# hpgmg/hpgmg

Hardware: AMD Instinct MI355X
Metric: DOF/s (fine-grid) for FMG F-cycle (higher is better)
Workload: dtype f64

## Files before the change

### hpgmg_amd/csrc/host/mg.c

```c
#include <stdio.h>
#include <stdlib.h>
#include <string.h>
#include <math.h>
#include <time.h>
#include <stdint.h>
#include "hpgmg_level.h"
#include "hpgmg_operators.h"
#include "hpgmg_mg.h"

hpgmg_solve_record hpgmg_last_solve;
int hpgmg_verbose = 1;

void hpgmg_communicator_free(communicator_type *C);

static double now(void) {
  struct timespec ts;
  clock_gettime(CLOCK_MONOTONIC, &ts);
  return (double)ts.tv_sec + 1e-9 * (double)ts.tv_nsec;
}
#define SAY(rank, ...) do { if ((rank) == 0 && hpgmg_verbose) { fprintf(stdout, __VA_ARGS__); fflush(stdout); } } while (0)

typedef struct { int send_rank, send_id, send_box, recv_rank, recv_id, recv_box, i, j, k; } xfer_t;

static int xfer_cmp(const void *pa, const void *pb) {
// ... 632 lines not shown
}
void MGPreconditionerApply(mg_type *G, int onLevel, int z_id, int r_id, double a, double b) {
  level_type *L = G->levels[onLevel];
  if (!L->active) return;
  L->vcycles_from_this_level++;
  zero_vector(L, z_id);
  MGVCycle(G, z_id, r_id, a, b, onLevel);
  seg_close();
}

static int hpgmg_fmg_vcycles = 0;
void hpgmg_set_fmg_vcycles(int n) { hpgmg_fmg_vcycles = n > 0 ? n : 0; }
static int fmg_zero_u_first = 0;
void hpgmg_fmg_zero_u_first(void) { fmg_zero_u_first = 1; }
static void fmg_solve_once(mg_type *G, int onLevel, int u_id, int F_id, double a, double b, double rtol);
void FMGSolve(mg_type *G, int onLevel, int u_id, int F_id, double a, double b, double rtol) {
  int attempt, l, booked[64];
  for (attempt = 0; attempt < 2; attempt++) {
    for (l = 0; l < G->num_levels && l < 64; l++) booked[l] = G->levels[l]->vcycles_from_this_level;
    hpgmg_solve_attempt_begin();
    fmg_solve_once(G, onLevel, u_id, F_id, a, b, rtol);
    if (!hpgmg_solve_attempt_end()) return;
    G->MGSolves_performed--;
    for (l = 0; l < G->num_levels && l < 64; l++) G->levels[l]->vcycles_from_this_level = booked[l];
    if (G->levels[onLevel]->active) zero_vector(G->levels[onLevel], u_id);
  }
  fprintf(stderr, "hpgmg: FMGSolve failed twice\n");
  exit(1);
}
static void fmg_solve_once(mg_type *G, int onLevel, int u_id, int F_id, double a, double b, double rtol) {
  const int e_id = u_id, R_id = VECTOR_R, maxVCycles = hpgmg_fmg_vcycles;
  const int bottom = G->num_levels - 1;
  level_type *L = G->levels[onLevel];
  char label[64];
  int l, v;
  int u_to_zero = fmg_zero_u_first;
  hpgmg_tick t;
  fmg_zero_u_first = 0;
  G->MGSolves_performed++;
  if (!L->active) return;
  SAY(L->my_rank, "FMGSolve... ");
  const double t0 = now();
  seg_reset(G, onLevel, u_id, F_id, a, b);

  t = hpgmg_tick_begin(L, &L->timers.Total, "norm(F), R = F");
  double norm_of_F = 0.0;
  int first_restriction = onLevel;
  int norm_deferred = 0;
  const hpgmg_fmg_hook *hook = fmg_hook;
  if (!hook && onLevel < bottom && hpgmg_norm_scale_restrict_fused_deferred(L, F_id, R_id, G->levels[onLevel + 1])) { first_restriction = onLevel + 1; norm_deferred = 1; }
  else if (!hook && onLevel < bottom && hpgmg_norm_scale_restrict_fused(L, F_id, R_id, G->levels[onLevel + 1], &norm_of_F)) first_restriction = onLevel + 1;
  else {
    norm_of_F = norm(L, F_id);
    scale_vector(L, R_id, 1.0, F_id);
  }
  hpgmg_tick_end(t);

  int ftail = bottom;
  for (l = onLevel; l < bottom && !hook; l++) if (is_small(G, l) && hpgmg_vcycle_legs_fused(&G->levels[l], G->num_levels - l, e_id, R_id, a, b, HPGMG_LEG_FCYCLE_TAIL_ASK)) { ftail = l; break; }

  if (u_to_zero && ftail <= onLevel) { zero_vector(L, u_id); u_to_zero = 0; }
  for (l = first_restriction; l < ftail; l++) {
    if (is_small(G, l)) seg_open();
    t = hpgmg_tick_begin(G->levels[l], &G->levels[l]->timers.Total, "restrict R");
    restriction(G->levels[l + 1], R_id, G->levels[l], R_id, RESTRICT_CELL);
    if (hook) hook->rhs_restricted(hook, G, l + 1, R_id);
    hpgmg_tick_end(t);
  }

  if (ftail < bottom) {
    if (is_small(G, ftail)) seg_open();
    t = hpgmg_tick_begin(G->levels[ftail], &G->levels[ftail]->timers.Total, "F-cycle tail (fused)");
    if (!hpgmg_vcycle_legs_fused(&G->levels[ftail], G->num_levels - ftail, e_id, R_id, a, b, HPGMG_LEG_FCYCLE_TAIL)) { fprintf(stderr, "fused F-cycle tail refused after being accepted\n"); exit(1); }
    hpgmg_tick_end(t);
// ... 79 lines not shown
```

### hpgmg_amd/csrc/host/operators_hip.c

```c
#include "plugin_internal.h"

void hp_do_restriction(level_type *Lc, int id_c, level_type *Lf, int id_f, int type) {
  TICK(Lf, restriction_total, "restriction");
  hp_coef_written(Lc, id_c);
  communicator_type *S = &Lf->restriction[type], *R = &Lc->restriction[type];
  backend_t *Bc = hp_backend_of(Lc), *Bf = hp_backend_of(Lf);
  HIP_OK(hpgmg_hip_restrict_blocks(&Bc->dev, id_c, &Bf->dev, id_f, hp_mirror(Lf, S->blocks[0], S->num_blocks[0]), S->num_blocks[0], type));
  hp_transport_phase(R, S, (Lf->tag << 4) | 0x5);
  HIP_OK(hpgmg_hip_restrict_blocks(&Bc->dev, id_c, &Bf->dev, id_f, hp_mirror(Lf, S->blocks[1], S->num_blocks[1]), S->num_blocks[1], type));
  HIP_OK(hpgmg_hip_copy_blocks(&Bc->dev, id_c, hp_mirror(Lc, R->blocks[2], R->num_blocks[2]), R->num_blocks[2]));
  TOCK();
}

int hpgmg_restrict_zero_fused(level_type *Lc, int id_c, level_type *Lf, int id_f, int zero_id) {
  communicator_type *S = &Lf->restriction[RESTRICT_CELL], *R = &Lc->restriction[RESTRICT_CELL];
  if (!Lf->active || !Lc->active || Lc->num_my_boxes < 1 || zero_id == id_c) return 0;
  if (S->num_sends || R->num_recvs || S->num_blocks[0] || R->num_blocks[2] || S->num_blocks[1] < 1) return 0;
  TICK(Lf, restriction_total, "restriction + zero_vector");
  backend_t *Bc = hp_backend_of(Lc), *Bf = hp_backend_of(Lf);
  HIP_OK(hpgmg_hip_restrict_cell_and_zero(&Bc->dev, id_c, &Bf->dev, id_f, hp_mirror(Lf, S->blocks[1], S->num_blocks[1]), S->num_blocks[1], zero_id));
  TOCK();
  return 1;
}

// ... 125 lines not shown
    if (B) { TICK(L, blas1, "norm(F), this rank's part (reduction deferred)"); HIP_OK(hpgmg_hip_norm_max(&B->dev, F_id, &v)); TOCK(); }
    hp_do_scale_vector(L, R_id, 1.0, F_id);
    hp_do_restriction(Lc, R_id, L, R_id, RESTRICT_CELL);
    deferred_host_value = v; deferred_on_device = 0;
  }
  deferred_norm_level = L;
  return 1;
}
double hpgmg_norm_deferred_fetch(level_type *L) {
  double v = deferred_host_value;
  if (deferred_norm_level != L) { fprintf(stderr, "hpgmg: no deferred norm is pending on this level\n"); abort(); }
  deferred_norm_level = NULL;
  if (deferred_on_device) HIP_OK(hpgmg_hip_deferred_fetch(&v));
  return hp_allreduce_scalar(L, v, HPGMG_REDUCE_MAX);
}
int hpgmg_residual_norm_fused(level_type *L, int res_id, int x_id, int rhs_id, double a, double b, double *norm_out) {
  hpgmg_config cfg;
  hpgmg_get_config(&cfg);
  if (cfg.op != HPGMG_OP_7PT && res_id >= 0) return 0;
  if (!L->active || L->num_my_boxes < 1) return 0;
  backend_t *B = hp_backend_of(L);
  const int ready = fused_residual_operand(L, B, x_id);
  if (!ready) return 0;
  double v = 0.0;
  { TICK(L, residual, "residual + norm (fused)");
    FUSED_LAUNCH(B, ready, hpgmg_hip_residual_norm(hp_stencil_dev(B), hp_variant(), res_id, x_id, rhs_id, a, b, 1.0 / (L->h * L->h), &v));
    TOCK(); }
  *norm_out = hp_allreduce_scalar(L, v, HPGMG_REDUCE_MAX);
  return 1;
}
// ... 129 lines not shown
```

### hpgmg_amd/csrc/host/plugin_internal.h

```cpp
#ifndef HPGMG_PLUGIN_INTERNAL_H
#define HPGMG_PLUGIN_INTERNAL_H
#include <stdio.h>
#include <stdlib.h>
#include <string.h>
#include <math.h>
#include <time.h>
#include <stdint.h>
#include "hpgmg_level.h"
#include "hpgmg_operators.h"
#include "hpgmg_mg.h"
#include "hpgmg_hip.h"

int hpgmg_smooth_sweeps(void);
int hpgmg_gsrb_out_of_place(void);

#define HP_INTERNAL __attribute__((visibility("hidden")))

enum { TIMERS_HOST = 0, TIMERS_DEVICE = 1, TIMERS_SYNC = 2 };
#define TICK(L, FIELD, WHAT) const hpgmg_tick tick_ = hpgmg_tick_begin((L), &(L)->timers.FIELD, WHAT)
#define TOCK() hpgmg_tick_end(tick_)
HP_INTERNAL void hp_lazy_flush(void);
#define HIP_OK(call) do { hp_lazy_flush(); int e_ = (call); if (e_) { fprintf(stderr, "hpgmg: %s failed (%d): %s\n", #call, e_, hpgmg_hip_last_error()); abort(); } } while (0)

#define MAX_LISTS 32
// ... 56 lines not shown
  double *storage, *scratch;
  double **d_box_base, **d_pair_base; int *d_box_low, *d_box_nbr;
  hpgmg_hip_level dev, dev_all;
  image_plan plan[IMG_PLANS];
  double *sendbuf, *recvbuf; size_t send_cap, recv_cap;
  double **ptr_tmp; int ptr_cap;
  hpgmg_hip_bc_entry *d_bc; int n_bc, n_bc_own;
  hpgmg_hip_bc_entry *d_bc_k; int n_bc_k;
  int *d_special; int n_special;
  int coef_valid, shape;
  double *seen_v0; int seen_nv;
} halo_images;

typedef enum { SW_GHOST_FREE = 0, SW_ONE_LAUNCH_GHOSTS, SW_OVERLAP, SW_PAIR_REMOTE, SW_IMAGES, SW_FUSED_SWEEPS, SW_PAIR_MIN_CELLS, SW_FUSED_RESIDUAL, SW_FUSED_TAIL,
               SW_FUSED_FTAIL, SW_FUSED_BOTTOM, SW_SMALL_FUSED, SW_SMALL_VTAIL, SW_SMALL_27PT_GSRB, SW_SMALL_OPS, SW_LAZY, SW_LAZY_REPORT, SW_TEMP_SCRATCH,
               SW_FV4_NO_EXACT_RB, SW_GRAPH, SW_SMOOTHER_PRECISION, SW_DEFER_NORM, SW_BRICK_VISITS, SW_BRICK_SIZE, SW_BRICK_MIN_DIM, SW_BRICK_FSTEP, SW_BRICK_CHAIN, SW_BRICK_WIDE, SW_BRICK_WIDE_MAX_DIM, SW_BRICK_WIDE_TAIL_DIM, SW_FTAIL_MAX_DIM, SW_PAIR_FORM_DINV, SW_UNIFORM_ALPHA, SW_COUNT } hp_switch_id;
HP_INTERNAL long long hp_switch(hp_switch_id id);
HP_INTERNAL void hp_switch_set(hp_switch_id id, long long value);

HP_INTERNAL backend_t *hp_backend_of(level_type *L);
HP_INTERNAL const blockCopy_type *hp_mirror(level_type *owner, const blockCopy_type *host, int n);
HP_INTERNAL int  hp_variant(void);
typedef struct { int kind, zero_first; } hp_small_bc;
HP_INTERNAL hp_small_bc hp_small_bc_rule(int op, const level_type *L);
HP_INTERNAL int  hp_boxes_lexicographic(level_type *L);
static inline int hp_comm_no_messages(const communicator_type *C) { return C->num_sends + C->num_recvs == 0 && !C->num_blocks[0] && !C->num_blocks[2]; }
static inline int hp_comm_nothing_to_exchange(const communicator_type *C) { return hp_comm_no_messages(C) && !C->num_blocks[1]; }
HP_INTERNAL int *hp_krylov_pinned(backend_t *B);
HP_INTERNAL int  hp_ghost_free_mode(void);
HP_INTERNAL backend_t *hp_pcg_backend(level_type *L);
HP_INTERNAL int  hp_box_rank_at(const level_type *L, int bi, int bj, int bk);
// ... 85 lines not shown
```

### hpgmg_amd/csrc/host/plugin_switches.c

```c
#include "plugin_internal.h"

enum { K_ON = 0, K_OFF = 1, K_INT = 2, K_TRI = 3 };
static struct { const char *env; int kind; long long dflt; const char *what; long long value; int known; } table[SW_COUNT] = {
  [SW_GHOST_FREE]        = { "HPGMG_GHOST_FREE", K_ON, 1, "stencil launches read neighbouring boxes and the Dirichlet rule themselves; 0: the reference's exchange + boundary + stencil launches" },
  [SW_ONE_LAUNCH_GHOSTS] = { "HPGMG_ONE_LAUNCH_GHOSTS", K_ON, 1, "27-pt / fv2 / fv4: box-to-box ghost copies and boundary conditions as one launch" },
  [SW_OVERLAP]           = { "HPGMG_OVERLAP", K_ON, 1, "N > 1: halo exchanges on a second stream under the part of the stencil launch that does not need them" },
  [SW_PAIR_REMOTE]       = { "HPGMG_PAIR_REMOTE", K_ON, 1, "N > 1, 7-pt: sweep pairs across rank boundaries (two-deep halo, one exchange per pair); 0: one exchange per sweep" },
  [SW_IMAGES]            = { "HPGMG_IMAGES", K_ON, 1, "N > 1, 27-pt / fv4: images of the neighbouring ranks' boxes (one-pass red + black kernels keep running); 0: exchange_boundary per half sweep" },
  [SW_FUSED_SWEEPS]      = { "HPGMG_FUSED_SWEEPS", K_ON, 1, "7-pt: two smoother sweeps per pass on bandwidth-bound levels" },
  [SW_PAIR_MIN_CELLS]    = { "HPGMG_PAIR_MIN_CELLS", K_INT, 2000000, "7-pt: smallest level (cells) that takes the sweep-pair kernel (2 M: the 128^3 level too, since the kernel picks its launch shape per launch -- 16 workgroup rows of 10 waves x 16 chunks = 256 workgroups there: config 2 2.70 vs 2.74 ms; with 16 waves it lost, 3.02 vs 2.92: profiles/r06k_ab_pair_min.txt, r06n_ab_pair_min.txt)" },
  [SW_FUSED_RESIDUAL]    = { "HPGMG_FUSED_RESIDUAL", K_ON, 1, "residual + restriction (+ zero_vector), residual + norm, norm + copy + restriction as one pass each" },
  [SW_FUSED_TAIL]        = { "HPGMG_FUSED_TAIL", K_ON, 1, "7-pt: the V-cycle below the brick levels (<= 8^3; <= 16^3 without them) as one single-workgroup launch" },
  [SW_FUSED_FTAIL]       = { "HPGMG_FUSED_FTAIL", K_ON, 1, "7-pt: the F-cycle's own work below 32^3 as one launch" },
  [SW_FUSED_BOTTOM]      = { "HPGMG_FUSED_BOTTOM", K_ON, 1, "BiCGStab bottom solve on the device; 0: driven from the host (host/solvers.c) through the operators" },
  [SW_SMALL_FUSED]       = { "HPGMG_SMALL_FUSED", K_TRI, 2, "27-pt / fv2 / fv4: smooth() of a one-box level as one launch on an LDS image (2, default); 0 off" },
  [SW_SMALL_VTAIL]       = { "HPGMG_SMALL_VTAIL", K_TRI, 2, "27-pt / fv2 / fv4: the V-cycle below a one-box level as one launch: 2 on except for 27-pt GSRB (default), 1 on, 0 off" },
  [SW_SMALL_27PT_GSRB]   = { "HPGMG_TUNE_SMALL_27PT_GSRB", K_OFF, 0, "27-pt GSRB: the one-launch small-level smooth() instead of the one-workgroup-per-box red + black kernel" },
  [SW_SMALL_OPS]         = { "HPGMG_SMALL_OPS", K_ON, 1, "BLAS-1 / operator calls of a host-driven Krylov solver on a small one-box level go out with the scalar that follows them" },
  [SW_LAZY]              = { "HPGMG_LAZY", K_ON, 1, "void operators are postponed while they follow MGVCycle's call order and issued fused (the reference's own driver, INTEGRATION.md Route B)" },
  [SW_LAZY_REPORT]       = { "HPGMG_LAZY_REPORT", K_OFF, 0, "print what the operator queue did when the process ends" },
  [SW_TEMP_SCRATCH]      = { "HPGMG_TEMP_SCRATCH", K_ON, 1, "inside a cycle VECTOR_TEMP is scratch after smooth(): in-cycle smoother forms; 0: the exact state of smooth() everywhere" },
  [SW_FV4_NO_EXACT_RB]   = { "HPGMG_TUNE_FV4_NO_EXACT_RB", K_OFF, 0, "fv4: the exported smooth() as six half sweeps (no red + black passes)" },
  [SW_GRAPH]             = { "HPGMG_GRAPH", K_OFF, 0, "capture / replay the launch-bound segments as hipGraphs (measured slower with a full stream)" },
  [SW_DEFER_NORM]        = { "HPGMG_DEFER_NORM", K_ON, 1, "FMGSolve: norm(F) of the opening pass is collected at the end, where it is used, instead of waited for at the start" },
  [SW_BRICK_VISITS]     = { "HPGMG_BRICK_VISITS", K_ON, 1, "7-pt: the 64^3 / 32^3 / 16^3 levels of a V-cycle leg as one launch of 8^3 bricks that trade faces, residuals and corrections inside the launch; 0 when other processes run such launches on the same GPU" },
  [SW_BRICK_SIZE]       = { "HPGMG_TUNE_BRICK", K_INT, 8, "side of those bricks: 8 (512 lanes, one cell each) or 16 (1024 lanes, four cells each)" },
  [SW_BRICK_MIN_DIM]    = { "HPGMG_TUNE_BRICK_MIN", K_INT, 16, "smallest level (cells per side) visited as bricks; the levels below it are the single-workgroup tail's" },
  [SW_BRICK_FSTEP]      = { "HPGMG_TUNE_BRICK_FSTEP", K_ON, 1, "FMGSolve: interpolation_fcycle onto a brick level rides in the first launch of the V-cycle that follows it" },
  [SW_BRICK_CHAIN]      = { "HPGMG_TUNE_BRICK_CHAIN", K_INT, 1, "consecutive brick levels of a V-cycle leg in ONE launch (what passes between the levels passes inside it); 0: one launch per level visit" },
  [SW_BRICK_WIDE]       = { "HPGMG_BRICK_WIDE", K_ON, 1, "27-pt / fv4: the same for the operators with wide stencils (kernels/brick_wide.hip: halo of the stencil's radius, apply_BCs_p2 / _v4 on the LDS image)" },
  [SW_BRICK_WIDE_MAX_DIM] = { "HPGMG_TUNE_BRICK_WIDE_MAX", K_INT, 64, "largest level (cells per side) the 27-pt / fv4 plugins visit as bricks (measured: fv4 `7 64` 29.71 / 29.91 / 30.15 ms with 64 / 32 / 16, 27-pt 12.27 / 12.51 / 12.52)" },
  [SW_BRICK_WIDE_TAIL_DIM] = { "HPGMG_TUNE_BRICK_WIDE_TAIL", K_INT, 1, "27-pt / fv4: the largest one-box level left to the single-workgroup tail (1: the 8^3, 4^3 (and 27-pt: 2^3) levels are visited as ONE brick each and only the bottom solve is left; 2 / 4 / 8: the tail starts there)" },
  [SW_FTAIL_MAX_DIM]    = { "HPGMG_TUNE_FTAIL_MAX", K_INT, 8, "7-pt: the largest level (cells per side) the single-launch F-cycle tail starts from (8: the 16^3 step of the climb is a brick launch each way, eight CUs instead of one: config 1 0.320 vs 0.328 ms with 16, config 2 the same within noise; profiles/r06i_ab_ftail.txt)" },
  [SW_PAIR_FORM_DINV]    = { "HPGMG_PAIR_FORM_DINV", K_ON, 1, "7-pt sweep pairs (fp64 streams, one rank, variable coefficients, 10 / 12 waves): Dinv is formed in registers from the coefficient streams instead of read, where VECTOR_DINV is known to be rebuild_operator's output for the same a, b; 0: always read" },
  [SW_UNIFORM_ALPHA]     = { "HPGMG_UNIFORM_ALPHA", K_ON, 1, "7-pt Helmholtz, one rank: where rebuild_operator found alpha to be one bit pattern over the level's interior, the sweep pairs that form Dinv and the wide fused residual passes take it from their arguments instead of streaming VECTOR_ALPHA; 0: always read" },
  [SW_SMOOTHER_PRECISION]= { "HPGMG_SMOOTHER_PRECISION", K_INT, 64, "32: fp32 coefficient streams in the Chebyshev sweep pairs (BASELINE config 5: within 2e-4 of the fp64 norms, and bit-exact against the CPU oracle's fp32 mode, which rounds the same coefficients); 64: bit-exact" },
};

long long hp_switch(hp_switch_id id) {
  if (!table[id].known) {
    const char *e = getenv(table[id].env);
    long long v = table[id].dflt;
    switch (table[id].kind) {
      case K_ON:  v = !(e && e[0] == '0'); break;
      case K_OFF: v = (e && e[0] == '1'); break;
      case K_INT: if (e && *e) v = atoll(e); break;
      default:    v = (e && e[0] == '0') ? 0 : ((e && e[0] == '1') ? 1 : table[id].dflt); break;
    }
    table[id].value = v; table[id].known = 1;
  }
// ... 11 lines not shown
```

### hpgmg_amd/csrc/kernels/blas1.hip

```cpp
#include "reduce.hpp"
#include "knobs.hpp"
#include "launch_dispatch.hpp"

namespace hpgmg {

constexpr int kRowsPerBlock = 4;

struct RowIter {
  int box, j, k;
};
__device__ __forceinline__ bool row_of(int row, int side, int num_boxes, RowIter &r) {
  const int per_box = side * side;
  if (row >= per_box * num_boxes) return false;
  r.box = row / per_box;
  const int rem = row - r.box * per_box;
  r.k = rem / side;
  r.j = rem - r.k * side;
  return true;
}
static inline int rows_grid(int rows) { return (rows + kRowsPerBlock - 1) / kRowsPerBlock; }

enum { OP_AXPBY = 0, OP_MUL, OP_INVERT, OP_SCALE, OP_SHIFT, OP_COLOR, OP_RANDOM };
struct EwArgs { int id_c, id_a, id_b; double sa, sb; int colors, ic, jc, kc; };

// ... 108 lines not shown
    for (int ci = lane; ci < half; ci += 64) {
      const double2 a = *reinterpret_cast<const double2 *>(f + 2 * ci), b = *reinterpret_cast<const double2 *>(f + 2 * ci + jS);
      const double2 cc = *reinterpret_cast<const double2 *>(f + 2 * ci + kS), d = *reinterpret_cast<const double2 *>(f + 2 * ci + jS + kS);
      const double2 ra = make_double2(1.0 * a.x, 1.0 * a.y), rb = make_double2(1.0 * b.x, 1.0 * b.y);
      const double2 rc = make_double2(1.0 * cc.x, 1.0 * cc.y), rd = make_double2(1.0 * d.x, 1.0 * d.y);
      store_pair<NT>(r + 2 * ci, ra); store_pair<NT>(r + 2 * ci + jS, rb);
      store_pair<NT>(r + 2 * ci + kS, rc); store_pair<NT>(r + 2 * ci + jS + kS, rd);
      double v = ra.x + ra.y; v = v + rb.x; v = v + rb.y; v = v + rc.x; v = v + rc.y; v = v + rd.x; v = v + rd.y;
      c[ci] = v * 0.125;
      double q;
      q = fabs(a.x); m = (q > m) ? q : m;  q = fabs(a.y); m = (q > m) ? q : m;  q = fabs(b.x); m = (q > m) ? q : m;  q = fabs(b.y); m = (q > m) ? q : m;
      q = fabs(cc.x); m = (q > m) ? q : m; q = fabs(cc.y); m = (q > m) ? q : m; q = fabs(d.x); m = (q > m) ? q : m;  q = fabs(d.y); m = (q > m) ? q : m;
    }
  }
  block_max_store(m, partials, blockIdx.x);
}

template <bool kFinish>
__global__ __launch_bounds__(64) void tile_sum_kernel(const hpgmg_hip_level L, int id_a, int id_b, double *partials, ResultSlot *result, unsigned long long seq) {
  __shared__ double part[64];
  const int tiles_side = (L.dim + BLOCKCOPY_TILE_J - 1) / BLOCKCOPY_TILE_J;
  const int tiles_per_box = tiles_side * tiles_side;
  const int ntiles = tiles_per_box * L.num_boxes;
  const int t = blockIdx.x * 64 + threadIdx.x;
  if (kFinish) part[threadIdx.x] = 0.0;
  if (t >= ntiles) { if (kFinish) __syncthreads(); return; }
  const int box = t / tiles_per_box, rem = t % tiles_per_box;
  const int k0 = (rem / tiles_side) * BLOCKCOPY_TILE_K, j0 = (rem % tiles_side) * BLOCKCOPY_TILE_J;
  const int k1 = min(k0 + BLOCKCOPY_TILE_K, L.dim), j1 = min(j0 + BLOCKCOPY_TILE_J, L.dim);
  const double *pa = vec_origin(L, box, id_a);
// ... 157 lines not shown
      Aii[i] = 1.0 / d;
    }
  }
  block_max_store(best, partials, blockIdx.x);
}

template <int OP>
static int launch_ew(const hpgmg_hip_level *L, const EwArgs &A) {
  HPGMG_SKIP_IF_REPLAY();
  if (L->num_boxes <= 0) return 0;
  const int rows = L->num_boxes * L->dim * L->dim;
  hipLaunchKernelGGL((elementwise_kernel<OP>), dim3(rows_grid(rows)), dim3(256), 0, g_stream, *L, A);
  HPGMG_LAUNCH_CHECK("elementwise_kernel");
  return 0;
}

}
using namespace hpgmg;

extern "C" {
int hpgmg_hip_graph_flush(void);

int hpgmg_hip_fill(const hpgmg_hip_level *L, int id, double v) {
  HPGMG_SKIP_IF_REPLAY();
  if (L->num_boxes <= 0) return 0;
  const int side = L->dim + 2 * L->ghosts, rows = L->num_boxes * side * side;
  hipLaunchKernelGGL(fill_kernel, dim3(rows_grid(rows)), dim3(256), 0, g_stream, *L, id, v);
  HPGMG_LAUNCH_CHECK("fill_kernel");
  return 0;
}
// ... 36 lines not shown
  if (int e = hpgmg_hip_graph_flush()) return e;
  if (norm_out) *norm_out = 0.0;
  if (L->num_boxes <= 0 || Lc->num_boxes <= 0 || (L->dim & 1) || !(L->flags & 1) || (L->jStride & 1) || (L->kStride & 1) || (L->volume & 1) || f_id == r_id)
    return record_error(hipErrorInvalidValue, "norm_copy_restrict: level not supported");
  const int nblk = rows_grid(L->num_boxes * (L->dim / 2) * (L->dim / 2));
  double *partials = reduction_scratch(nblk);
  if (!partials) return record_error(hipErrorOutOfMemory, "norm_copy_restrict: no scratch");
  if (knob(K_COPY_NT) && (double)L->num_boxes * L->dim * L->dim * L->dim * sizeof(double) > 256e6)
    hipLaunchKernelGGL(norm_copy_restrict_kernel<true>, dim3(nblk), dim3(256), 0, g_stream, *L, f_id, r_id, *Lc, rc_id, map, partials);
  else hipLaunchKernelGGL(norm_copy_restrict_kernel<false>, dim3(nblk), dim3(256), 0, g_stream, *L, f_id, r_id, *Lc, rc_id, map, partials);
  HPGMG_LAUNCH_CHECK("norm_copy_restrict");
  if (!norm_out) return 0;
  if (!deferred) return max_of_partials(nblk, 0.0, norm_out);
  if (int e = scalar_begin(&g_deferred, true)) return e;
  return max_of_partials(nblk, 0.0, g_deferred);
}
int hpgmg_hip_norm_max(const hpgmg_hip_level *L, int id, double *out) {
  if (int e = hpgmg_hip_graph_flush()) return e;
  *out = 0.0;
  if (L->num_boxes <= 0) return 0;
  const int nblk = rows_grid(L->num_boxes * L->dim * L->dim);
  if (nblk <= 64) {
    Scalar t;
    if (int e = scalar_begin(&t)) return e;
    hipLaunchKernelGGL(absmax_small_kernel, dim3(1), dim3(256), 0, g_stream, *L, id, t.slot, t.seq);
    HPGMG_LAUNCH_CHECK("norm_max");
    return scalar_wait(t, out);
  }
  int per_box = rows_grid(L->dim * L->dim);
  while (per_box > 1 && (long long)per_box * L->num_boxes > 4096) per_box = (per_box + 1) / 2;
// ... 76 lines not shown
```

### include/hpgmg_fv.h

```cpp
#ifndef HPGMG_FV_H
#define HPGMG_FV_H

#include "hpgmg_level.h"
#include "hpgmg_operators.h"
#include "hpgmg_mg.h"

#ifdef __cplusplus
extern "C" {
#endif

typedef struct hpgmg_solver {
  level_type level_h;
  mg_type    mg;
  double a, b, h;
  int boxes_in_i, box_dim;
  int my_rank, num_ranks;
} hpgmg_solver;

int hpgmg_choose_boxes_in_i(int log2_box_dim, int target_boxes_per_rank, int num_ranks);

hpgmg_solver *hpgmg_solver_create(int log2_box_dim, int target_boxes_per_rank, int bc, int my_rank, int num_ranks);
hpgmg_solver *hpgmg_solver_create_explicit(int boxes_in_i, int box_dim, int bc, int my_rank, int num_ranks);
void hpgmg_solver_destroy(hpgmg_solver *s);

// ... 89 lines not shown
long long   hpgmg_small_ops_prefetched(void);
void        hpgmg_set_fused_bottom(int on);
void        hpgmg_set_fused_tail(int on);
void        hpgmg_set_brick_visits(int on);
long long   hpgmg_brick_visits(void);
long long   hpgmg_brick_failures(void);
long long   hpgmg_brick_capacity_refusals(void);
void        hpgmg_set_brick_wide(int on);
void        hpgmg_set_brick_chains(int on);
long long   hpgmg_pair_remote_smooths(void);
long long   hpgmg_fp32_pair_smooths(void);
void        hpgmg_set_pair_form_dinv(int on);
long long   hpgmg_pair_formed_dinv_launches(void);
void        hpgmg_set_uniform_alpha(int on);
long long   hpgmg_uniform_alpha_launches(void);
long long   hpgmg_fused_residuals_remote(void);
long long   hpgmg_fv4_rb_smooths(void);
long long   hpgmg_rb27_passes(void);
long long   hpgmg_image_exchanges(void);
void        hpgmg_level_timers(level_type *level, double out[9]);
void        hpgmg_set_gather_dim(int dim);
long long   hpgmg_overlap_count(void);
void        hpgmg_set_overlap(int on);
void        hpgmg_set_smoother_precision(int bits);
int         hpgmg_get_smoother_precision(void);
void        hpgmg_set_graphs(int on);
void        hpgmg_set_fused_sweeps(int on);
void        hpgmg_set_pair_min_cells(long long cells);
void        hpgmg_set_ghost_free(int on);
void        hpgmg_set_box_alignment(int jstride, int kstride, int volume, int base_bytes);
// ... 6 lines not shown
```

### include/hpgmg_hip.h

```cpp
#ifndef HPGMG_HIP_H
#define HPGMG_HIP_H

#include <stddef.h>
#include "hpgmg_level.h"

#ifdef __cplusplus
extern "C" {
#endif

typedef struct {
  double *const *box_base;
  const int *box_low;
  int num_boxes;
  int dim, ghosts, jStride, kStride, volume;
  int dim_i, dim_j, dim_k;
  int periodic;
  const int *box_nbr;
  int flags;
  long long box_stride;
} hpgmg_hip_level;

enum { HPGMG_HIP_7PT_VC_HELMHOLTZ = 0, HPGMG_HIP_7PT_VC_POISSON = 1, HPGMG_HIP_7PT_CC = 2,
       HPGMG_HIP_27PT_CC = 3, HPGMG_HIP_FV4_VC_HELMHOLTZ = 4, HPGMG_HIP_FV4_VC_POISSON = 5 };

// ... 153 lines not shown
                                 const blockCopy_type *blocks, int num_blocks, int order);

int hpgmg_hip_fill(const hpgmg_hip_level *L, int id, double interior_value);
int hpgmg_hip_axpby(const hpgmg_hip_level *L, int id_c, double sa, int id_a, double sb, int id_b);
int hpgmg_hip_mul(const hpgmg_hip_level *L, int id_c, double s, int id_a, int id_b);
int hpgmg_hip_invert(const hpgmg_hip_level *L, int id_c, double s, int id_a);
int hpgmg_hip_scale(const hpgmg_hip_level *L, int id_c, double s, int id_a);
int hpgmg_hip_shift(const hpgmg_hip_level *L, int id_c, int id_a, double shift);
int hpgmg_hip_color(const hpgmg_hip_level *L, int id, int colors, int ic, int jc, int kc);
int hpgmg_hip_random(const hpgmg_hip_level *L, int id);
int hpgmg_hip_norm_max(const hpgmg_hip_level *L, int id, double *out);
int hpgmg_hip_dot(const hpgmg_hip_level *L, int id_a, int id_b, double *out);
int hpgmg_hip_norm_copy_restrict(const hpgmg_hip_level *L, int f_id, int r_id, const hpgmg_hip_level *Lc, int rc_id, const int *map, double *norm_out);
int  hpgmg_hip_norm_copy_restrict_deferred(const hpgmg_hip_level *L, int f_id, int r_id, const hpgmg_hip_level *Lc, int rc_id, const int *restrict_map);
int  hpgmg_hip_deferred_fetch(double *out);
int hpgmg_hip_sum(const hpgmg_hip_level *L, int id, double *out);
int hpgmg_hip_gram(const hpgmg_hip_level *L, const int *id_A, int rows, const int *id_B, int cols, double *C_host);
int hpgmg_hip_pcg_supported(const hpgmg_hip_level *L, int variant);
int hpgmg_hip_pcg_apply_dot(const hpgmg_hip_level *L, int variant, int Ap_id, int p_id, double a, double b, double h2inv, double *dot);
int hpgmg_hip_pcg_update(const hpgmg_hip_level *L, int x_id, int r_id, int p_id, int Ap_id, double alpha, double *rmax);
int hpgmg_hip_pcg_dot(const hpgmg_hip_level *L, int a_id, int b_id, double *dot);
int hpgmg_hip_pcg_dot2(const hpgmg_hip_level *L, int a_id, int c_id, int b_id, double *ab, double *cb);
#define HPGMG_HIP_BLOCK_TILE 6
int hpgmg_hip_block_supported(const hpgmg_hip_level *L);
int hpgmg_hip_block_tile(void);
int hpgmg_hip_block_gram(const hpgmg_hip_level *L, const int *a_ids, int na, const int *b_ids, int nb, int w_id, double *G_host);
int hpgmg_hip_block_combine(const hpgmg_hip_level *L, const int *out_ids, int nout, const int *in_ids, int nin, const double *C_host);
int hpgmg_hip_block_residual(const hpgmg_hip_level *L, const int *r_ids, const int *ax_ids, const int *x_ids, int n, int w_id, const double *mu,
                             double *rmax, double *mxmax);

// ... 96 lines not shown
```

### include/hpgmg_operators.h

```cpp
#ifndef HPGMG_OPERATORS_H
#define HPGMG_OPERATORS_H

#include "hpgmg_level.h"

#ifdef __cplusplus
extern "C" {
#endif

#define VECTOR_TEMP    0
#define VECTOR_U       1
#define VECTOR_F       2
#define VECTOR_E       3
#define VECTOR_R       4
#define VECTOR_DINV    5
#define VECTOR_BETA_I  6
#define VECTOR_BETA_J  7
#define VECTOR_BETA_K  8
#define VECTOR_ALPHA   9
#define VECTOR_L1INV  10

enum { HPGMG_OP_7PT = 0, HPGMG_OP_27PT = 1, HPGMG_OP_FV4 = 2, HPGMG_OP_FV2 = 3 };
enum { HPGMG_SMOOTH_CHEBY = 0, HPGMG_SMOOTH_GSRB = 1, HPGMG_SMOOTH_JACOBI = 2 };

typedef struct {
// ... 116 lines not shown
int     hpgmg_solve_attempt_end(void);
int     hpgmg_bottom_solve_fused(level_type *L, int e_id, int R_id, double a, double b, double desired_reduction_in_norm);
int     hpgmg_interp_smooth_fused(level_type *fine, int e_id, int R_id, level_type *coarse, double a, double b);
int     hpgmg_restrict_zero_fused(level_type *coarse, int id_c, level_type *fine, int id_f, int zero_id);
typedef struct { double t0; double *acc; int slot, range; } hpgmg_tick;
hpgmg_tick hpgmg_tick_begin(level_type *level, double *acc_seconds, const char *what);
void    hpgmg_tick_end(hpgmg_tick t);
void    hpgmg_timers_settle(void);
void    hpgmg_set_timer_mode(int mode);
int     hpgmg_get_timer_mode(void);
int     hpgmg_residual_restrict_zero_fused(level_type *coarse, int id_c, level_type *fine, int x_id, int rhs_id, double a, double b, int zero_id);
int     hpgmg_residual_norm_fused(level_type *level, int res_id, int x_id, int rhs_id, double a, double b, double *norm_out);
int     hpgmg_norm_scale_restrict_fused(level_type *level, int F_id, int R_id, level_type *coarse, double *norm_out);
int     hpgmg_norm_scale_restrict_fused_deferred(level_type *level, int F_id, int R_id, level_type *coarse);
double  hpgmg_norm_deferred_fetch(level_type *level);
int     hpgmg_zero_interpolation_fcycle_fused(level_type *fine, int id_f, level_type *coarse, int id_c);
int     hpgmg_smooth_in_cycle(level_type *level, int phi_id, int rhs_id, double a, double b);
void    hpgmg_operators_flush(void);
void    hpgmg_set_lazy(int on);
void    hpgmg_level_sync_counters(level_type *level);
void    hpgmg_level_release(level_type *level);
const char *hpgmg_backend_name(void);

#ifdef __cplusplus
}
#endif
#endif
```

Before: 7.590 billion.

## Fuse norm, copy and multi-level restriction of F into one cascade launch

The opening FMG pass over F (max-norm, R = F copy, restriction to the next level) now also carries the restricted values down up to four coarser levels inside one kernel, using shared memory per block tile. This removes several separate restriction launches and the coarse-level re-reads they cause at the start of each F-cycle. The F-cycle tail probe is moved earlier so the cascade depth can stop at the fused tail. In exchange the kernel is larger and uses more shared memory, and it only applies on one rank with aligned restriction maps.

```diff
diff --git a/hpgmg_amd/csrc/host/mg.c b/hpgmg_amd/csrc/host/mg.c
--- a/hpgmg_amd/csrc/host/mg.c
+++ b/hpgmg_amd/csrc/host/mg.c
@@ -670,6 +670,7 @@
 static int fmg_zero_u_first = 0;
 void hpgmg_fmg_zero_u_first(void) { fmg_zero_u_first = 1; }
 static void fmg_solve_once(mg_type *G, int onLevel, int u_id, int F_id, double a, double b, double rtol);
+extern int hpgmg_norm_scale_restrict_cascade(level_type **levels, int max_depth, int F_id, int R_id, double *norm_out, int *norm_deferred) __attribute__((weak));
 void FMGSolve(mg_type *G, int onLevel, int u_id, int F_id, double a, double b, double rtol) {
   int attempt, l, booked[64];
   for (attempt = 0; attempt < 2; attempt++) {
@@ -699,21 +700,24 @@
   const double t0 = now();
   seg_reset(G, onLevel, u_id, F_id, a, b);
 
+  const hpgmg_fmg_hook *hook = fmg_hook;
+  int ftail = bottom;
+  for (l = onLevel; l < bottom && !hook; l++) if (is_small(G, l) && hpgmg_vcycle_legs_fused(&G->levels[l], G->num_levels - l, e_id, R_id, a, b, HPGMG_LEG_FCYCLE_TAIL_ASK)) { ftail = l; break; }
+
   t = hpgmg_tick_begin(L, &L->timers.Total, "norm(F), R = F");
   double norm_of_F = 0.0;
   int first_restriction = onLevel;
   int norm_deferred = 0;
-  const hpgmg_fmg_hook *hook = fmg_hook;
-  if (!hook && onLevel < bottom && hpgmg_norm_scale_restrict_fused_deferred(L, F_id, R_id, G->levels[onLevel + 1])) { first_restriction = onLevel + 1; norm_deferred = 1; }
+  int cascade = 0;
+  if (!hook && ftail > onLevel && hpgmg_norm_scale_restrict_cascade) cascade = hpgmg_norm_scale_restrict_cascade(&G->levels[onLevel], ftail - onLevel, F_id, R_id, &norm_of_F, &norm_deferred);
+  if (cascade > 0) first_restriction = onLevel + cascade;
+  else if (!hook && onLevel < bottom && hpgmg_norm_scale_restrict_fused_deferred(L, F_id, R_id, G->levels[onLevel + 1])) { first_restriction = onLevel + 1; norm_deferred = 1; }
   else if (!hook && onLevel < bottom && hpgmg_norm_scale_restrict_fused(L, F_id, R_id, G->levels[onLevel + 1], &norm_of_F)) first_restriction = onLevel + 1;
   else {
     norm_of_F = norm(L, F_id);
     scale_vector(L, R_id, 1.0, F_id);
   }
   hpgmg_tick_end(t);
-
-  int ftail = bottom;
-  for (l = onLevel; l < bottom && !hook; l++) if (is_small(G, l) && hpgmg_vcycle_legs_fused(&G->levels[l], G->num_levels - l, e_id, R_id, a, b, HPGMG_LEG_FCYCLE_TAIL_ASK)) { ftail = l; break; }
 
   if (u_to_zero && ftail <= onLevel) { zero_vector(L, u_id); u_to_zero = 0; }
   for (l = first_restriction; l < ftail; l++) {
diff --git a/hpgmg_amd/csrc/host/operators_hip.c b/hpgmg_amd/csrc/host/operators_hip.c
--- a/hpgmg_amd/csrc/host/operators_hip.c
+++ b/hpgmg_amd/csrc/host/operators_hip.c
@@ -163,6 +163,70 @@
   if (deferred_on_device) HIP_OK(hpgmg_hip_deferred_fetch(&v));
   return hp_allreduce_scalar(L, v, HPGMG_REDUCE_MAX);
 }
+static long long restrict_cascade_launches = 0, restrict_cascade_levels = 0;
+long long hpgmg_restrict_cascade_launches(void) { return restrict_cascade_launches; }
+long long hpgmg_restrict_cascade_levels(void) { return restrict_cascade_levels; }
+void hpgmg_set_restrict_cascade(int on) {
+  hp_lazy_flush(); hpgmg_hip_graph_reset();
+  hp_switch_set(SW_RESTRICT_CASCADE, on ? 1 : 0);
+}
+static int cascade_map_aligned(level_type *Lf, int unit) {
+  communicator_type *S = &Lf->restriction[RESTRICT_CELL];
+  int n;
+  for (n = 0; n < S->num_blocks[1]; n++) {
+    const blockCopy_type *e = &S->blocks[1][n];
+    if ((e->write.i - e->read.i / 2) % unit || (e->write.j - e->read.j / 2) % unit || (e->write.k - e->read.k / 2) % unit) return 0;
+  }
+  return 1;
+}
+static int restrict_cascade_depth(level_type **levels, int max_depth) {
+  const hpgmg_transport *T = hpgmg_get_transport();
+  int d = 0, l;
+  if (!fused_residual_on() || !hp_switch(SW_RESTRICT_CASCADE) || (T && T->size > 1)) return 0;
+  if (max_depth > 4) max_depth = 4;
+  for (l = 0; l < max_depth; l++) {
+    level_type *Lf = levels[l], *Lc = levels[l + 1];
+    communicator_type *S = &Lf->restriction[RESTRICT_CELL], *R = &Lc->restriction[RESTRICT_CELL];
+    if (!Lf->active || !Lc->active || Lf->num_my_boxes < 1 || Lc->num_my_boxes < 1) break;
+    if (S->num_sends || R->num_recvs || S->num_blocks[0] || R->num_blocks[2] || S->num_blocks[1] < 1) break;
+    if ((Lf->box_dim & 1) || Lf->box_dim < (l ? 2 : 16)) break;
+    if (!restrict_map_of(Lf, hp_backend_of(Lf))) break;
+    d = l + 1;
+  }
+  for (; d > 0; d--) {
+    if (!hpgmg_hip_norm_copy_restrict_cascade_supported(&hp_backend_of(levels[0])->dev, d)) continue;
+    for (l = 0; l < d - 1; l++) if (!cascade_map_aligned(levels[l], 1 << (d - 1 - l))) break;
+    if (l >= d - 1) break;
+  }
+  return d;
+}
+int hpgmg_restrict_cascade_depth(level_type **levels, int max_depth) { return restrict_cascade_depth(levels, max_depth); }
+int hpgmg_norm_scale_restrict_cascade(level_type **levels, int max_depth, int F_id, int R_id, double *norm_out, int *norm_deferred) {
+  const hpgmg_hip_level *dev[5];
+  const int *maps[4];
+  level_type *L = levels[0];
+  int l;
+  if (F_id == R_id || max_depth < 1) return 0;
+  const int d = restrict_cascade_depth(levels, max_depth);
+  if (d < 1) return 0;
+  hp_lazy_flush();
+  for (l = 0; l <= d; l++) {
+    dev[l] = &hp_backend_of(levels[l])->dev;
+    if (l < d) maps[l] = hp_backend_of(levels[l])->d_restrict_map;
+    if (l) hp_coef_written(levels[l], R_id);
+  }
+  hp_coef_written(L, R_id);
+  const int defer = (int)hp_switch(SW_DEFER_NORM);
+  double v = 0.0;
+  { TICK(L, blas1, "norm(F) + R = F + restrictions (one launch)");
+    HIP_OK(hpgmg_hip_norm_copy_restrict_cascade(dev, F_id, R_id, R_id, maps, d, &v, defer));
+    TOCK(); }
+  restrict_cascade_launches++; restrict_cascade_levels += d;
+  if (defer) { deferred_norm_level = L; deferred_on_device = 1; }
+  else *norm_out = hp_allreduce_scalar(L, v, HPGMG_REDUCE_MAX);
+  *norm_deferred = defer;
+  return d;
+}
 int hpgmg_residual_norm_fused(level_type *L, int res_id, int x_id, int rhs_id, double a, double b, double *norm_out) {
   hpgmg_config cfg;
   hpgmg_get_config(&cfg);
diff --git a/hpgmg_amd/csrc/host/plugin_internal.h b/hpgmg_amd/csrc/host/plugin_internal.h
--- a/hpgmg_amd/csrc/host/plugin_internal.h
+++ b/hpgmg_amd/csrc/host/plugin_internal.h
@@ -94,7 +94,7 @@
 
 typedef enum { SW_GHOST_FREE = 0, SW_ONE_LAUNCH_GHOSTS, SW_OVERLAP, SW_PAIR_REMOTE, SW_IMAGES, SW_FUSED_SWEEPS, SW_PAIR_MIN_CELLS, SW_FUSED_RESIDUAL, SW_FUSED_TAIL,
                SW_FUSED_FTAIL, SW_FUSED_BOTTOM, SW_SMALL_FUSED, SW_SMALL_VTAIL, SW_SMALL_27PT_GSRB, SW_SMALL_OPS, SW_LAZY, SW_LAZY_REPORT, SW_TEMP_SCRATCH,
-               SW_FV4_NO_EXACT_RB, SW_GRAPH, SW_SMOOTHER_PRECISION, SW_DEFER_NORM, SW_BRICK_VISITS, SW_BRICK_SIZE, SW_BRICK_MIN_DIM, SW_BRICK_FSTEP, SW_BRICK_CHAIN, SW_BRICK_WIDE, SW_BRICK_WIDE_MAX_DIM, SW_BRICK_WIDE_TAIL_DIM, SW_FTAIL_MAX_DIM, SW_PAIR_FORM_DINV, SW_UNIFORM_ALPHA, SW_COUNT } hp_switch_id;
+               SW_FV4_NO_EXACT_RB, SW_GRAPH, SW_SMOOTHER_PRECISION, SW_DEFER_NORM, SW_BRICK_VISITS, SW_BRICK_SIZE, SW_BRICK_MIN_DIM, SW_BRICK_FSTEP, SW_BRICK_CHAIN, SW_BRICK_WIDE, SW_BRICK_WIDE_MAX_DIM, SW_BRICK_WIDE_TAIL_DIM, SW_FTAIL_MAX_DIM, SW_PAIR_FORM_DINV, SW_UNIFORM_ALPHA, SW_RESTRICT_CASCADE, SW_COUNT } hp_switch_id;
 HP_INTERNAL long long hp_switch(hp_switch_id id);
 HP_INTERNAL void hp_switch_set(hp_switch_id id, long long value);
 
diff --git a/hpgmg_amd/csrc/host/plugin_switches.c b/hpgmg_amd/csrc/host/plugin_switches.c
--- a/hpgmg_amd/csrc/host/plugin_switches.c
+++ b/hpgmg_amd/csrc/host/plugin_switches.c
@@ -34,6 +34,7 @@
   [SW_FTAIL_MAX_DIM]    = { "HPGMG_TUNE_FTAIL_MAX", K_INT, 8, "7-pt: the largest level (cells per side) the single-launch F-cycle tail starts from (8: the 16^3 step of the climb is a brick launch each way, eight CUs instead of one: config 1 0.320 vs 0.328 ms with 16, config 2 the same within noise; profiles/r06i_ab_ftail.txt)" },
   [SW_PAIR_FORM_DINV]    = { "HPGMG_PAIR_FORM_DINV", K_ON, 1, "7-pt sweep pairs (fp64 streams, one rank, variable coefficients, 10 / 12 waves): Dinv is formed in registers from the coefficient streams instead of read, where VECTOR_DINV is known to be rebuild_operator's output for the same a, b; 0: always read" },
   [SW_UNIFORM_ALPHA]     = { "HPGMG_UNIFORM_ALPHA", K_ON, 1, "7-pt Helmholtz, one rank: where rebuild_operator found alpha to be one bit pattern over the level's interior, the sweep pairs that form Dinv and the wide fused residual passes take it from their arguments instead of streaming VECTOR_ALPHA; 0: always read" },
+  [SW_RESTRICT_CASCADE]  = { "HPGMG_RESTRICT_CASCADE", K_ON, 1, "FMGSolve, one rank: the opening pass over F (norm + copy + restriction) also carries the restricted R down the levels below it, up to four, in the one launch; 0: one level, the other restrictions launch by launch" },
   [SW_SMOOTHER_PRECISION]= { "HPGMG_SMOOTHER_PRECISION", K_INT, 64, "32: fp32 coefficient streams in the Chebyshev sweep pairs (BASELINE config 5: within 2e-4 of the fp64 norms, and bit-exact against the CPU oracle's fp32 mode, which rounds the same coefficients); 64: bit-exact" },
 };
 
diff --git a/hpgmg_amd/csrc/kernels/blas1.hip b/hpgmg_amd/csrc/kernels/blas1.hip
--- a/hpgmg_amd/csrc/kernels/blas1.hip
+++ b/hpgmg_amd/csrc/kernels/blas1.hip
@@ -146,6 +146,89 @@
     }
   }
   block_max_store(m, partials, blockIdx.x);
+}
+
+constexpr int kCascadeMaxDepth = 4, kCascadeThreads = 512, kCascadeMaxI = 128, kCascadeMaxE = 16;
+struct CascadeArgs {
+  hpgmg_hip_level lv[kCascadeMaxDepth + 1];
+  const int *map[kCascadeMaxDepth];
+  int f_id, r_id, rc_id, block_i, block_e;
+};
+struct CascadeCell { double2 a, b, c, d; };
+__device__ __forceinline__ CascadeCell cascade_load(const double *f, int jS, int kS) {
+  CascadeCell q;
+  q.a = *reinterpret_cast<const double2 *>(f); q.b = *reinterpret_cast<const double2 *>(f + jS);
+  q.c = *reinterpret_cast<const double2 *>(f + kS); q.d = *reinterpret_cast<const double2 *>(f + jS + kS);
+  return q;
+}
+template <bool NT> __device__ __forceinline__ double cascade_cell(const CascadeCell &q, double *r, int jS, int kS, double &m) {
+  const double2 ra = make_double2(1.0 * q.a.x, 1.0 * q.a.y), rb = make_double2(1.0 * q.b.x, 1.0 * q.b.y);
+  const double2 rc = make_double2(1.0 * q.c.x, 1.0 * q.c.y), rd = make_double2(1.0 * q.d.x, 1.0 * q.d.y);
+  store_pair<NT>(r, ra); store_pair<NT>(r + jS, rb); store_pair<NT>(r + kS, rc); store_pair<NT>(r + jS + kS, rd);
+  double v = ra.x + ra.y; v = v + rb.x; v = v + rb.y; v = v + rc.x; v = v + rc.y; v = v + rd.x; v = v + rd.y;
+  double t;
+  t = fabs(q.a.x); m = (t > m) ? t : m;  t = fabs(q.a.y); m = (t > m) ? t : m;  t = fabs(q.b.x); m = (t > m) ? t : m;  t = fabs(q.b.y); m = (t > m) ? t : m;
+  t = fabs(q.c.x); m = (t > m) ? t : m;  t = fabs(q.c.y); m = (t > m) ? t : m;  t = fabs(q.d.x); m = (t > m) ? t : m;  t = fabs(q.d.y); m = (t > m) ? t : m;
+  return v * 0.125;
+}
+__device__ __forceinline__ void cascade_level(const double *src, int si, int se, double *dst, double *c, int jSc, int kSc) {
+  const int di = si >> 1, de = se >> 1, n = di * de * de, rj = si, rk = si * se;
+  for (int t = (int)threadIdx.x; t < n; t += kCascadeThreads) {
+    const int i = t % di, row = t / di, j = row % de, k = row / de;
+    const double *f = src + 2 * i + 2 * j * rj + 2 * k * rk;
+    double v = f[0] + f[1]; v = v + f[rj]; v = v + f[1 + rj]; v = v + f[rk]; v = v + f[1 + rk]; v = v + f[rj + rk]; v = v + f[1 + rj + rk];
+    v = v * 0.125;
+    c[i + j * jSc + k * kSc] = v;
+    if (dst) dst[t] = v;
+  }
+}
+template <int DEPTH, bool NT>
+__global__ __launch_bounds__(kCascadeThreads) void norm_copy_restrict_cascade_kernel(const CascadeArgs A, double *partials) {
+  __shared__ double s1[(kCascadeMaxI / 2) * (kCascadeMaxE / 2) * (kCascadeMaxE / 2)];
+  __shared__ double s2[(kCascadeMaxI / 4) * (kCascadeMaxE / 4) * (kCascadeMaxE / 4)], s3[(kCascadeMaxI / 8) * (kCascadeMaxE / 8) * (kCascadeMaxE / 8)];
+  __shared__ double smax[kCascadeThreads / 64];
+  const hpgmg_hip_level &L = A.lv[0];
+  const int bi = A.block_i, be = A.block_e, per_i = L.dim / bi, per_e = L.dim / be, tid = (int)threadIdx.x;
+  int b = (int)blockIdx.x;
+  const int ib = b % per_i; b /= per_i;
+  const int jb = b % per_e; b /= per_e;
+  const int kb = b % per_e;
+  int box = b / per_e, oi = ib * bi, oj = jb * be, ok = kb * be;
+  const int jS = L.jStride, kS = L.kStride;
+  const double *f = vec_origin(L, box, A.f_id) + oi + oj * jS + ok * kS;
+  double *r = vec_origin(L, box, A.r_id) + oi + oj * jS + ok * kS;
+  double *c;
+  int jSc, kSc;
+  auto descend = [&](int l) {
+    const int *mp = A.map[l] + 4 * box;
+    const hpgmg_hip_level &Lc = A.lv[l + 1];
+    box = mp[0]; oi = mp[1] + (oi >> 1); oj = mp[2] + (oj >> 1); ok = mp[3] + (ok >> 1);
+    jSc = Lc.jStride; kSc = Lc.kStride;
+    c = vec_origin(Lc, box, A.rc_id) + oi + oj * jSc + ok * kSc;
+  };
+  descend(0);
+  const int hi = bi >> 1, he = be >> 1, n1 = hi * he * he, she = __builtin_ctz(he);
+  double m = 0.0;
+  for (int t0 = tid; t0 < n1; t0 += 2 * kCascadeThreads) {
+    const int t1 = t0 + kCascadeThreads;
+    const bool two = t1 < n1;
+    const int ci0 = t0 % hi, row0 = t0 / hi, cj0 = row0 & (he - 1), ck0 = row0 >> she;
+    const int u1 = two ? t1 : t0, ci1 = u1 % hi, row1 = u1 / hi, cj1 = row1 & (he - 1), ck1 = row1 >> she;
+    const int off0 = 2 * ci0 + 2 * cj0 * jS + 2 * ck0 * kS, off1 = 2 * ci1 + 2 * cj1 * jS + 2 * ck1 * kS;
+    const CascadeCell q0 = cascade_load(f + off0, jS, kS), q1 = cascade_load(f + off1, jS, kS);
+    const double v0 = cascade_cell<NT>(q0, r + off0, jS, kS, m);
+    c[ci0 + cj0 * jSc + ck0 * kSc] = v0;
+    if (DEPTH > 1) s1[t0] = v0;
+    if (two) {
+      const double v1 = cascade_cell<NT>(q1, r + off1, jS, kS, m);
+      c[ci1 + cj1 * jSc + ck1 * kSc] = v1;
+      if (DEPTH > 1) s1[t1] = v1;
+    }
+  }
+  if (DEPTH > 1) { __syncthreads(); descend(1); cascade_level(s1, bi >> 1, be >> 1, DEPTH > 2 ? s2 : nullptr, c, jSc, kSc); }
+  if (DEPTH > 2) { __syncthreads(); descend(2); cascade_level(s2, bi >> 2, be >> 2, DEPTH > 3 ? s3 : nullptr, c, jSc, kSc); }
+  if (DEPTH > 3) { __syncthreads(); descend(3); cascade_level(s3, bi >> 3, be >> 3, nullptr, c, jSc, kSc); }
+  block_max_store<kCascadeThreads / 64>(m, smax, partials, blockIdx.x);
 }
 
 template <bool kFinish>
@@ -333,6 +416,11 @@
   HPGMG_LAUNCH_CHECK("elementwise_kernel");
   return 0;
 }
+template <int DEPTH>
+static void cascade_launch(bool nt, int nblk, const CascadeArgs &A, double *partials) {
+  if (nt) hipLaunchKernelGGL((norm_copy_restrict_cascade_kernel<DEPTH, true>), dim3(nblk), dim3(kCascadeThreads), 0, g_stream, A, partials);
+  else hipLaunchKernelGGL((norm_copy_restrict_cascade_kernel<DEPTH, false>), dim3(nblk), dim3(kCascadeThreads), 0, g_stream, A, partials);
+}
 
 }
 using namespace hpgmg;
@@ -399,6 +487,46 @@
   if (!deferred) return max_of_partials(nblk, 0.0, norm_out);
   if (int e = scalar_begin(&g_deferred, true)) return e;
   return max_of_partials(nblk, 0.0, g_deferred);
+}
+static int cascade_block(const hpgmg_hip_level *L, int depth, int *block_e) {
+  if (depth < 1 || depth > kCascadeMaxDepth || L->num_boxes <= 0 || L->dim <= 0 || (L->dim & ((1 << depth) - 1))) return 0;
+  if (!(L->flags & 1) || (L->jStride & 1) || (L->kStride & 1) || (L->volume & 1)) return 0;
+  const int bi = (L->dim <= kCascadeMaxI) ? L->dim : ((L->dim % kCascadeMaxI) ? 0 : kCascadeMaxI);
+  *block_e = (L->dim % kCascadeMaxE) ? (1 << depth) : kCascadeMaxE;
+  return bi;
+}
+int hpgmg_hip_norm_copy_restrict_cascade_supported(const hpgmg_hip_level *L, int depth) { int be; return cascade_block(L, depth, &be) > 0; }
+int hpgmg_hip_norm_copy_restrict_cascade(const hpgmg_hip_level *const *levels, int f_id, int r_id, int rc_id, const int *const *maps, int depth, double *norm_out, int deferred) {
+  if (int e = hpgmg_hip_graph_flush()) return e;
+  if (norm_out) *norm_out = 0.0;
+  if (depth < 1 || depth > kCascadeMaxDepth || !levels || !maps || !levels[0]) return record_error(hipErrorInvalidValue, "norm_copy_restrict_cascade: depth not supported");
+  CascadeArgs A = {};
+  A.block_i = cascade_block(levels[0], depth, &A.block_e);
+  if (!A.block_i || f_id == r_id) return record_error(hipErrorInvalidValue, "norm_copy_restrict_cascade: level not supported");
+  for (int l = 0; l <= depth; l++) {
+    if (!levels[l] || levels[l]->num_boxes <= 0 || (l < depth && !maps[l])) return record_error(hipErrorInvalidValue, "norm_copy_restrict_cascade: level not supported");
+    A.lv[l] = *levels[l];
+    if (l < depth) A.map[l] = maps[l];
+  }
+  A.f_id = f_id; A.r_id = r_id; A.rc_id = rc_id;
+  const hpgmg_hip_level *L = levels[0];
+  const int per_e = L->dim / A.block_e, nblk = L->num_boxes * (L->dim / A.block_i) * per_e * per_e;
+  double *partials = reduction_scratch(nblk);
+  if (!partials) return record_error(hipErrorOutOfMemory, "norm_copy_restrict_cascade: no scratch");
+  const bool nt = knob(K_COPY_NT) && (double)L->num_boxes * L->dim * L->dim * L->dim * sizeof(double) > 256e6;
+  switch (depth) {
+    case 1: cascade_launch<1>(nt, nblk, A, partials); break;
+    case 2: cascade_launch<2>(nt, nblk, A, partials); break;
+    case 3: cascade_launch<3>(nt, nblk, A, partials); break;
+    default: cascade_launch<4>(nt, nblk, A, partials); break;
+  }
+  HPGMG_LAUNCH_CHECK("norm_copy_restrict_cascade");
+  if (deferred) {
+    if (int e = scalar_begin(&g_deferred, true)) return e;
+    return max_of_partials(nblk, 0.0, g_deferred);
+  }
+  if (!norm_out) return 0;
+  return max_of_partials(nblk, 0.0, norm_out);
 }
 int hpgmg_hip_norm_max(const hpgmg_hip_level *L, int id, double *out) {
   if (int e = hpgmg_hip_graph_flush()) return e;
diff --git a/include/hpgmg_fv.h b/include/hpgmg_fv.h
--- a/include/hpgmg_fv.h
+++ b/include/hpgmg_fv.h
@@ -127,6 +127,9 @@
 long long   hpgmg_pair_formed_dinv_launches(void);
 void        hpgmg_set_uniform_alpha(int on);
 long long   hpgmg_uniform_alpha_launches(void);
+void        hpgmg_set_restrict_cascade(int on);
+long long   hpgmg_restrict_cascade_launches(void);
+long long   hpgmg_restrict_cascade_levels(void);
 long long   hpgmg_fused_residuals_remote(void);
 long long   hpgmg_fv4_rb_smooths(void);
 long long   hpgmg_rb27_passes(void);
diff --git a/include/hpgmg_hip.h b/include/hpgmg_hip.h
--- a/include/hpgmg_hip.h
+++ b/include/hpgmg_hip.h
@@ -191,6 +191,8 @@
 int hpgmg_hip_norm_copy_restrict(const hpgmg_hip_level *L, int f_id, int r_id, const hpgmg_hip_level *Lc, int rc_id, const int *map, double *norm_out);
 int  hpgmg_hip_norm_copy_restrict_deferred(const hpgmg_hip_level *L, int f_id, int r_id, const hpgmg_hip_level *Lc, int rc_id, const int *restrict_map);
 int  hpgmg_hip_deferred_fetch(double *out);
+int  hpgmg_hip_norm_copy_restrict_cascade_supported(const hpgmg_hip_level *L, int depth);
+int  hpgmg_hip_norm_copy_restrict_cascade(const hpgmg_hip_level *const *levels, int f_id, int r_id, int rc_id, const int *const *maps, int depth, double *norm_out, int deferred);
 int hpgmg_hip_sum(const hpgmg_hip_level *L, int id, double *out);
 int hpgmg_hip_gram(const hpgmg_hip_level *L, const int *id_A, int rows, const int *id_B, int cols, double *C_host);
 int hpgmg_hip_pcg_supported(const hpgmg_hip_level *L, int variant);
diff --git a/include/hpgmg_operators.h b/include/hpgmg_operators.h
--- a/include/hpgmg_operators.h
+++ b/include/hpgmg_operators.h
@@ -154,6 +154,8 @@
 int     hpgmg_norm_scale_restrict_fused(level_type *level, int F_id, int R_id, level_type *coarse, double *norm_out);
 int     hpgmg_norm_scale_restrict_fused_deferred(level_type *level, int F_id, int R_id, level_type *coarse);
 double  hpgmg_norm_deferred_fetch(level_type *level);
+int     hpgmg_norm_scale_restrict_cascade(level_type **levels, int max_depth, int F_id, int R_id, double *norm_out, int *norm_deferred);
+int     hpgmg_restrict_cascade_depth(level_type **levels, int max_depth);
 int     hpgmg_zero_interpolation_fcycle_fused(level_type *fine, int id_f, level_type *coarse, int id_c);
 int     hpgmg_smooth_in_cycle(level_type *level, int phi_id, int rhs_id, double a, double b);
 void    hpgmg_operators_flush(void);
```

Result: no change. 7.644 billion (median of 6 runs) (+0.7%).
